# Gautham-JS/ROS_Stereo_SLAM

Hardware: AMD Instinct MI355X
Metric: stereo frames/sec @1241x376, 4096 kpts (higher is better)
Workload: dtype u8/i32 fixed-point (LK) + f32/f64 (geometry)

## Files before the change

ros_stereo_slam_amd/csrc/anms.hip:

```cpp
#include <cfloat>

#include "svo_internal.h"
#include "wave_ops.hip.h"

namespace {


struct AnmsJob {
    const float2 *xy;
    const float *resp;
    int *order;
    float4 *sorted;
    double *radius, *decision;
    int *out_idx, *d_count;
    const float2 *in_a, *in_b;
    float2 *out_a, *out_b;
    const uint8_t *in_s;
    uint8_t *out_s;
    const int *gate;
};
template <int NJ> struct AnmsBatchN {
    AnmsJob j[NJ];
};
using AnmsBatch = AnmsBatchN<SVO_LK_MAX_JOBS>;

constexpr int KPW_GROUP = 8;
constexpr int KPW_LONE = 2;

template <int KPW> __global__ __launch_bounds__(64) void anms_rank_kernel(AnmsBatchN<KPW == KPW_LONE ? 1 : SVO_LK_MAX_JOBS> batch, int n)
{
    svo_chain_priority();
    const AnmsJob &job = batch.j[blockIdx.y];
    if (job.gate && *job.gate == 0)
        return;
    const float2 *__restrict__ xy = job.xy;
    const float *__restrict__ resp = job.resp;
    int *__restrict__ order = job.order;
    float4 *__restrict__ sorted = job.sorted;
    const int lane = threadIdx.x & 63;
    const int i0 = blockIdx.x * KPW;
    if (i0 >= n)
        return;
    float ri[KPW];
    int cnt[KPW];
#pragma unroll
    for (int q = 0; q < KPW; q++) {
        ri[q] = resp[min(i0 + q, n - 1)];
        cnt[q] = 0;
    }
    const float *__restrict__ rl = resp + lane;
    const int own = (i0 >> 6) << 6;
#pragma unroll 2
    for (int j0 = 0; j0 < own; j0 += 64) {
        const float rj = rl[j0];
#pragma unroll
        for (int q = 0; q < KPW; q++)
            cnt[q] += rj >= ri[q] ? 1 : 0;
    }
    {
        const int j = own + lane;
        if (j < n) {
            const float rj = rl[own];
#pragma unroll
            for (int q = 0; q < KPW; q++)
                cnt[q] += (rj > ri[q] || (rj == ri[q] && j < i0 + q)) ? 1 : 0;
        }
    }
    int j0 = own + 64;
#pragma unroll 2
    for (; j0 + 64 <= n; j0 += 64) {
        const float rj = rl[j0];
#pragma unroll
        for (int q = 0; q < KPW; q++)
            cnt[q] += rj > ri[q] ? 1 : 0;
    }
    if (j0 < n && j0 + lane < n) {
        const float rj = rl[j0];
#pragma unroll
        for (int q = 0; q < KPW; q++)
            cnt[q] += rj > ri[q] ? 1 : 0;
    }
#pragma unroll
    for (int q = 0; q < KPW; q++) {
        const int rank = svo::wave_sum_dpp(cnt[q]);
        if (lane == 0 && i0 + q < n) {
            order[rank] = i0 + q;
            const float2 p = xy[i0 + q];
            sorted[rank] = make_float4(p.x, p.y, ri[q], 0.f);
        }
    }
}

template <int KPW> __global__ __launch_bounds__(64) void anms_radius_kernel(AnmsBatchN<KPW == KPW_LONE ? 1 : SVO_LK_MAX_JOBS> batch, int n)
{
    svo_chain_priority();
    if (batch.j[blockIdx.y].gate && *batch.j[blockIdx.y].gate == 0)
        return;
    const float4 *__restrict__ sorted = batch.j[blockIdx.y].sorted;
    double *__restrict__ radius_sq = batch.j[blockIdx.y].radius;
    const int lane = threadIdx.x & 63;
    const int s0 = blockIdx.x * KPW;
    if (s0 >= n)
        return;
    float mx[KPW], my[KPW], thr[KPW];
    double best[KPW];
    unsigned active = 0;
#pragma unroll
    for (int q = 0; q < KPW; q++) {
        const float4 me = sorted[min(s0 + q, n - 1)];
        mx[q] = me.x;
        my[q] = me.y;
        thr[q] = me.z * 1.11f;
        best[q] = DBL_MAX;
        if (s0 + q < n && s0 + q > 0)
            active |= 1u << q;
    }
    for (int j0 = 0; j0 < s0 + KPW - 1 && active; j0 += 64) {
        const int j = j0 + lane;
        const float4 o = sorted[min(j, n - 1)];
#pragma unroll
        for (int q = 0; q < KPW; q++) {
            if (!((active >> q) & 1u))
                continue;
            bool dom = false;
            if (j < s0 + q) {
                dom = o.z > thr[q];
                if (dom) {
                    const float dx = mx[q] - o.x, dy = my[q] - o.y;
                    const double d = (double)dx * dx + (double)dy * dy;
                    best[q] = d < best[q] ? d : best[q];
                }
            }
            if (!__any(dom) || j0 + 64 >= s0 + q)
                active &= ~(1u << q);
        }
    }
#pragma unroll
    for (int q = 0; q < KPW; q++) {
        double b = best[q];
#pragma unroll
        for (int off = 32; off >= 1; off >>= 1) {
            const double o = __shfl_xor(b, off);
            b = o < b ? o : b;
        }
        if (lane == 0 && s0 + q < n)
            radius_sq[s0 + q] = b;
    }
}

template <int KPW> __global__ __launch_bounds__(64) void anms_decide_kernel(AnmsBatchN<KPW == KPW_LONE ? 1 : SVO_LK_MAX_JOBS> batch, int n, int keep)
{
    svo_chain_priority();
    if (batch.j[blockIdx.y].gate && *batch.j[blockIdx.y].gate == 0)
        return;
    const double *__restrict__ radius_sq = batch.j[blockIdx.y].radius;
    double *__restrict__ decision = batch.j[blockIdx.y].decision;
    const int lane = threadIdx.x & 63;
    const int s0 = blockIdx.x * KPW;
    if (s0 >= n)
        return;
    double ri[KPW];
    int gt[KPW], ge[KPW];
#pragma unroll
    for (int q = 0; q < KPW; q++) {
        ri[q] = radius_sq[min(s0 + q, n - 1)];
        gt[q] = ge[q] = 0;
    }
    const double *__restrict__ rl = radius_sq + lane;
    int j0 = 0;
#pragma unroll 2
    for (; j0 + 64 <= n; j0 += 64) {
        const double rj = rl[j0];
#pragma unroll
        for (int q = 0; q < KPW; q++) {
            gt[q] += rj > ri[q] ? 1 : 0;
            ge[q] += rj >= ri[q] ? 1 : 0;
        }
    }
    if (j0 + lane < n) {
        const double rj = rl[j0];
#pragma unroll
        for (int q = 0; q < KPW; q++) {
            gt[q] += rj > ri[q] ? 1 : 0;
            ge[q] += rj >= ri[q] ? 1 : 0;
        }
    }
#pragma unroll
    for (int q = 0; q < KPW; q++) {
        const int g = svo::wave_sum_dpp(gt[q]), e = svo::wave_sum_dpp(ge[q]);
        if (lane == 0 && s0 + q < n && g <= keep && keep < e)
            *decision = ri[q];
    }
}

constexpr int GATHER_T = 256;
template <int NJ> __global__ __launch_bounds__(GATHER_T) void anms_gather_kernel(AnmsBatchN<NJ> batch, int n)
{
    svo_chain_priority();
    const AnmsJob &job = batch.j[blockIdx.x];
    if (job.gate && *job.gate == 0)
        return;
    const double *__restrict__ radius_sq = job.radius;
    const double decision = *job.decision;
    const int *__restrict__ order = job.order;
    int *__restrict__ out_idx = job.out_idx;
    int *__restrict__ d_count = job.d_count;
    __shared__ int s_wave[GATHER_T / 64];
    const int t = threadIdx.x, lane = t & 63, wave = t >> 6;
    const int per = (n + GATHER_T - 1) / GATHER_T;
    const int b = t * per, e = min(b + per, n);
    int cnt = 0;
    for (int i = b; i < e; i++)
        cnt += radius_sq[i] >= decision ? 1 : 0;
    int incl = cnt;
#pragma unroll
    for (int off = 1; off < 64; off <<= 1) {
        const int o = __shfl_up(incl, off, 64);
        incl += lane >= off ? o : 0;
    }
    if (lane == 63)
        s_wave[wave] = incl;
    __syncthreads();
    int pos = incl - cnt, total = 0;
#pragma unroll
    for (int w2 = 0; w2 < GATHER_T / 64; w2++) {
        const int wt = s_wave[w2];
        pos += w2 < wave ? wt : 0;
        total += wt;
    }
    if (t == 0)
        *d_count = total;
    for (int i = b; i < e; i++)
        if (radius_sq[i] >= decision) {
            const int j = order[i];
            out_idx[pos] = j;
            if (job.out_a) {
                job.out_a[pos] = job.in_a[j];
                job.out_b[pos] = job.in_b[j];
                job.out_s[pos] = job.in_s[j];
            }
            pos++;
        }
}

template <int NJ> __global__ __launch_bounds__(64) void anms_payload_kernel(AnmsBatchN<NJ> batch, int n)
{
    const AnmsJob &job = batch.j[blockIdx.y];
    if (job.gate && *job.gate == 0)
        return;
    const int i = blockIdx.x * 64 + threadIdx.x;
    if (i == 0)
        *job.d_count = n;
    if (i >= n)
        return;
    const int j = job.order[i];
    job.out_idx[i] = j;
    if (!job.out_a)
        return;
    job.out_a[i] = job.in_a[j];
    job.out_b[i] = job.in_b[j];
    if (job.out_s)
        job.out_s[i] = job.in_s[j];
}

}

int svo_launch_anms_batch(svo_ctx *ctx, int k, const float *const *xy, const float *const *resp, int n, int keep,
                          int *const *out_idx, int *const *d_count, const svo_anms_gather *gather, const int *const *gates)
{
    if (n <= 0 || k <= 0)
        return SVO_OK;
    if (k > SVO_LK_MAX_JOBS) {
        svo_set_error("anms: at most %d jobs per launch", SVO_LK_MAX_JOBS);
        return SVO_ERR_ARG;
    }
    ScopedKernelTime tm(ctx, SVO_K_ANMS);
    int rc;
    const size_t na = ((size_t)n + 63) / 64 * 64;
    if ((rc = ctx->w_a.ensure(na * 4 * k)) || (rc = ctx->w_b.ensure((na * 8 + 64) * k)) ||
        (rc = ctx->w_d.ensure(na * 16 * k)))
        return rc;
    AnmsBatch batch;
    for (int a = 0; a < SVO_LK_MAX_JOBS; a++) {
        const int q = a < k ? a : 0;
        AnmsJob &j = batch.j[a];
        j.xy = reinterpret_cast<const float2 *>(xy[q]);
        j.resp = resp[q];
        j.order = ctx->w_a.as<int>() + na * q;
        j.radius = reinterpret_cast<double *>(ctx->w_b.as<uint8_t>() + (na * 8 + 64) * q);
        j.decision = j.radius + na;
        j.sorted = ctx->w_d.as<float4>() + na * q;
        j.out_idx = out_idx[q];
        j.d_count = d_count[q];
        j.in_a = gather ? reinterpret_cast<const float2 *>(gather[q].in_a) : nullptr;
        j.in_b = gather ? reinterpret_cast<const float2 *>(gather[q].in_b) : nullptr;
        j.out_a = gather ? reinterpret_cast<float2 *>(gather[q].out_a) : nullptr;
        j.out_b = gather ? reinterpret_cast<float2 *>(gather[q].out_b) : nullptr;
        j.in_s = gather ? gather[q].in_s : nullptr;
        j.out_s = gather ? gather[q].out_s : nullptr;
        j.gate = gates ? gates[q] : nullptr;
    }
    const bool lone = k == 1;
    const int kpw = lone ? KPW_LONE : KPW_GROUP;
    const dim3 wgrid((n + kpw - 1) / kpw, k), block(64);
    AnmsBatchN<1> one;
    one.j[0] = batch.j[0];
    if (lone)
        hipLaunchKernelGGL(anms_rank_kernel<KPW_LONE>, wgrid, block, 0, ctx->stream, one, n);
    else
        hipLaunchKernelGGL(anms_rank_kernel<KPW_GROUP>, wgrid, block, 0, ctx->stream, batch, n);
    if (n <= keep) {
        if (lone)
            hipLaunchKernelGGL(anms_payload_kernel<1>, dim3((n + 63) / 64, k), dim3(64), 0, ctx->stream, one, n);
        else
            hipLaunchKernelGGL(anms_payload_kernel<SVO_LK_MAX_JOBS>, dim3((n + 63) / 64, k), dim3(64), 0, ctx->stream, batch, n);
        SVO_HIP(hipGetLastError());
        return SVO_OK;
    }
    if (lone) {
        hipLaunchKernelGGL(anms_radius_kernel<KPW_LONE>, wgrid, block, 0, ctx->stream, one, n);
        hipLaunchKernelGGL(anms_decide_kernel<KPW_LONE>, wgrid, block, 0, ctx->stream, one, n, keep);
        hipLaunchKernelGGL(anms_gather_kernel<1>, dim3(k), dim3(GATHER_T), 0, ctx->stream, one, n);
    } else {
        hipLaunchKernelGGL(anms_radius_kernel<KPW_GROUP>, wgrid, block, 0, ctx->stream, batch, n);
        hipLaunchKernelGGL(anms_decide_kernel<KPW_GROUP>, wgrid, block, 0, ctx->stream, batch, n, keep);
        hipLaunchKernelGGL(anms_gather_kernel<SVO_LK_MAX_JOBS>, dim3(k), dim3(GATHER_T), 0, ctx->stream, batch, n);
    }
    SVO_HIP(hipGetLastError());
    return SVO_OK;
}

int svo_launch_anms(svo_ctx *ctx, const float *xy, const float *resp, int n, int keep, int *out_idx, int *d_count)
{
    return svo_launch_anms_batch(ctx, 1, &xy, &resp, n, keep, &out_idx, &d_count);
}

extern "C" int svo_anms(svo_ctx *ctx, const float *xy, const float *response, int n, int num_to_keep, int *out_idx,
                        int *count, int mem)
{
    SVO_CHECK_ARG(ctx && n >= 0 && num_to_keep >= 0);
    SVO_CHECK_ARG(mem == SVO_MEM_HOST || mem == SVO_MEM_DEVICE);
    if (n == 0) {
        if (count && mem == SVO_MEM_HOST)
            *count = 0;
        else if (count)
            SVO_HIP(hipMemsetAsync(count, 0, sizeof(int), ctx->stream));
        return SVO_OK;
    }
    SVO_CHECK_ARG(xy && response && out_idx && count);
    if (mem == SVO_MEM_DEVICE)
        return svo_launch_anms(ctx, xy, response, n, num_to_keep, out_idx, count);
    int rc;
    if ((rc = ctx->s_a.ensure((size_t)n * 8)) || (rc = ctx->s_b.ensure((size_t)n * 4)) ||
        (rc = ctx->s_c.ensure((size_t)n * 4 + 64)))
        return rc;
    SVO_HIP(hipMemcpyAsync(ctx->s_a.p, xy, (size_t)n * 8, hipMemcpyHostToDevice, ctx->stream));
    SVO_HIP(hipMemcpyAsync(ctx->s_b.p, response, (size_t)n * 4, hipMemcpyHostToDevice, ctx->stream));
    int *didx = ctx->s_c.as<int>(), *dcnt = didx + n;
    rc = svo_launch_anms(ctx, ctx->s_a.as<float>(), ctx->s_b.as<float>(), n, num_to_keep, didx, dcnt);
    if (rc)
        return rc;
    SVO_HIP(hipMemcpyAsync(ctx->pinned, dcnt, 4, hipMemcpyDeviceToHost, ctx->stream));
    SVO_HIP(hipStreamSynchronize(ctx->stream));
    const int k = *reinterpret_cast<int *>(ctx->pinned);
    SVO_HIP(hipMemcpyAsync(out_idx, didx, (size_t)k * 4, hipMemcpyDeviceToHost, ctx->stream));
    SVO_HIP(hipStreamSynchronize(ctx->stream));
    *count = k;
    return SVO_OK;
}
```

ros_stereo_slam_amd/csrc/context.hip:

```cpp
#include <cstdarg>

#include <cstdlib>
#include <chrono>
#include <cstdlib>
#include <thread>

#include "svo_internal.h"

static thread_local char g_err[512] = "";

void svo_set_error(const char *fmt, ...)
{
    va_list ap;
    va_start(ap, fmt);
    vsnprintf(g_err, sizeof(g_err), fmt, ap);
    va_end(ap);
}

int DevBuf::ensure(size_t bytes)
{
    if (bytes <= cap)
        return SVO_OK;
    if (p)
        (void)hipFree(p);
    p = nullptr;
    cap = 0;
    size_t want = bytes < 4096 ? 4096 : bytes + bytes / 4;
    hipError_t e = hipMalloc(&p, want);
    if (e != hipSuccess) {
        svo_set_error("hipMalloc(%zu) -> %s", want, hipGetErrorString(e));
        return SVO_ERR_HIP;
    }
    cap = want;
    return SVO_OK;
}

void DevBuf::release()
{
    if (p)
        (void)hipFree(p);
    p = nullptr;
    cap = 0;
}

ScopedKernelTime::ScopedKernelTime(svo_ctx *c, int kid) : ctx(c), id(kid)
{
    if (!ctx->timing)
        return;
    KernelTimer &t = ctx->timers[id];
    if (!t.pool.empty()) {
        a = t.pool.back().first;
        b = t.pool.back().second;
        t.pool.pop_back();
    } else {
        if (hipEventCreate(&a) != hipSuccess || hipEventCreate(&b) != hipSuccess) {
            a = b = nullptr;
            return;
        }
    }
    (void)hipEventRecord(a, ctx->stream);
}

ScopedKernelTime::~ScopedKernelTime()
{
    if (!a)
        return;
    (void)hipEventRecord(b, ctx->stream);
    ctx->timers[id].pending.emplace_back(a, b);
}

int svo_resolve_timers(svo_ctx *ctx)
{
    for (int k = 0; k < SVO_K_COUNT; k++) {
        KernelTimer &t = ctx->timers[k];
        for (auto &pr : t.pending) {
            float ms = 0.f;
            if (hipEventSynchronize(pr.second) == hipSuccess &&
                hipEventElapsedTime(&ms, pr.first, pr.second) == hipSuccess) {
                t.total_ms += ms;
                t.launches++;
            }
            t.pool.push_back(pr);
        }
        t.pending.clear();
    }
    return SVO_OK;
}

int svo_wait(svo_ctx *ctx) { return svo_wait_stream(ctx, ctx->stream); }

int svo_wait_stream(svo_ctx *ctx, hipStream_t stream)
{
    static const long spin_us = [] {
        const char *e = getenv("SVO_WAIT_SPIN_US");
        return e ? atol(e) : 300L;
    }();
    SVO_HIP(hipEventRecord(ctx->wait_ev, stream));
    const auto t0 = std::chrono::steady_clock::now();
    for (unsigned n = 0;; n++) {
        hipError_t e = hipEventQuery(ctx->wait_ev);
        if (e == hipSuccess)
            return SVO_OK;
        if (e != hipErrorNotReady) {
            svo_set_error("hipEventQuery -> %s", hipGetErrorString(e));
            return SVO_ERR_HIP;
        }
        if ((n & 15) != 15)
            continue;
        const long us = (long)std::chrono::duration_cast<std::chrono::microseconds>(std::chrono::steady_clock::now() - t0).count();
        if (us < spin_us)
            continue;
        if (us < spin_us + 2000)
            std::this_thread::yield();
        else
            std::this_thread::sleep_for(std::chrono::microseconds(50));
    }
}

extern "C" {

int svo_version(void) { return SVO_VERSION; }
const char *svo_last_error(void) { return g_err; }

int svo_ctx_create(int device, svo_ctx **out)
{
    SVO_CHECK_ARG(out != nullptr);
    *out = nullptr;
    int count = 0;
    hipError_t e = hipGetDeviceCount(&count);
    if (e != hipSuccess || count <= 0) {
        svo_set_error("no HIP device available (%s); libsvo_hip has no CPU fallback",
                      e == hipSuccess ? "device count 0" : hipGetErrorString(e));
        return SVO_ERR_NO_DEVICE;
    }
    SVO_CHECK_ARG(device >= 0 && device < count);
    SVO_HIP(hipSetDevice(device));
    hipDeviceProp_t prop;
    SVO_HIP(hipGetDeviceProperties(&prop, device));
    if (strncmp(prop.gcnArchName, "gfx950", 6) != 0) {
        svo_set_error("device %d is %s; this library carries gfx950 code objects only", device,
                      prop.gcnArchName);
        return SVO_ERR_NO_DEVICE;
    }
    svo_ctx *ctx = new svo_ctx();
    ctx->device = device;
    if (const char *pr = getenv("SVO_CTX_PRIORITY_EXPERIMENT"); pr && atoi(pr)) {
        int lo = 0, hi = 0;
        (void)hipDeviceGetStreamPriorityRange(&lo, &hi);
        e = hipStreamCreateWithPriority(&ctx->stream, hipStreamNonBlocking, atoi(pr) > 0 ? hi : lo);
    } else
        e = hipStreamCreateWithFlags(&ctx->stream, hipStreamNonBlocking);
    if (e != hipSuccess) {
        delete ctx;
        svo_set_error("hipStreamCreate -> %s", hipGetErrorString(e));
        return SVO_ERR_HIP;
    }
    ctx->pinned_bytes = 1 << 16;
    e = hipHostMalloc(&ctx->pinned, ctx->pinned_bytes, hipHostMallocDefault);
    if (e != hipSuccess) {
        (void)hipStreamDestroy(ctx->stream);
        delete ctx;
        svo_set_error("hipHostMalloc -> %s", hipGetErrorString(e));
        return SVO_ERR_HIP;
    }
    if (hipMalloc(reinterpret_cast<void **>(&ctx->d_tickets), SVO_N_TICKETS * sizeof(unsigned)) != hipSuccess ||
        hipMemset(ctx->d_tickets, 0, SVO_N_TICKETS * sizeof(unsigned)) != hipSuccess) {
        (void)hipHostFree(ctx->pinned);
        (void)hipStreamDestroy(ctx->stream);
        delete ctx;
        svo_set_error("hipMalloc(tickets) failed");
        return SVO_ERR_HIP;
    }
    e = hipEventCreateWithFlags(&ctx->wait_ev, hipEventDisableTiming);
    if (e != hipSuccess) {
        (void)hipHostFree(ctx->pinned);
        (void)hipStreamDestroy(ctx->stream);
        delete ctx;
        svo_set_error("hipEventCreate -> %s", hipGetErrorString(e));
        return SVO_ERR_HIP;
    }
    *out = ctx;
    return SVO_OK;
}

int svo_ctx_destroy(svo_ctx *ctx)
{
    if (!ctx)
        return SVO_OK;
    (void)hipSetDevice(ctx->device);
    (void)hipStreamSynchronize(ctx->stream);
    svo_resolve_timers(ctx);
    for (int k = 0; k < SVO_K_COUNT; k++)
        for (auto &pr : ctx->timers[k].pool) {
            (void)hipEventDestroy(pr.first);
            (void)hipEventDestroy(pr.second);
        }
    if (ctx->orb_cache)
        svo_orb_destroy(ctx->orb_cache);
    ctx->orb_cache = nullptr;
    if (ctx->orb_cv_cache)
        svo_orb_cv_destroy(ctx->orb_cv_cache);
    ctx->orb_cv_cache = nullptr;
    DevBuf *bufs[] = {&ctx->s_img, &ctx->s_a, &ctx->s_b, &ctx->s_c, &ctx->s_d, &ctx->s_e,
                      &ctx->s_f,   &ctx->s_g, &ctx->w_a, &ctx->w_b, &ctx->w_c, &ctx->w_d,
                      &ctx->w_e,   &ctx->orb_out, &ctx->orb_cv_out, &ctx->orb_cv_img, &ctx->orb_cv_ptrs,
                      &ctx->sgbm_cost, &ctx->sgbm_misc, &ctx->sgbm_rp, &ctx->sor_grid, &ctx->icp_work, &ctx->ess,
                      &ctx->feat_img, &ctx->feat_sum, &ctx->sift_pyr, &ctx->sift_work, &ctx->sift_out,
                      &ctx->brief_work, &ctx->brief_pat, &ctx->surf_planes, &ctx->surf_work,
                      &ctx->wls_work, &ctx->wls_maps, &ctx->wls_lut, &ctx->fast_work,
                      &ctx->voxel_work, &ctx->voxel_stage, &ctx->rect_stage};
    for (DevBuf *b : bufs)
        b->release();
    ctx->up_ring.release();
    for (int k = 0; k < 3; k++) {
        if (ctx->up_ev[k])
            (void)hipEventDestroy(ctx->up_ev[k]);
        if (ctx->use_ev[k])
            (void)hipEventDestroy(ctx->use_ev[k]);
    }
    if (ctx->up_stream)
        (void)hipStreamDestroy(ctx->up_stream);
    if (ctx->d_tickets)
        (void)hipFree(ctx->d_tickets);
    if (ctx->pinned)
        (void)hipHostFree(ctx->pinned);
    if (ctx->wait_ev)
        (void)hipEventDestroy(ctx->wait_ev);
    (void)hipStreamDestroy(ctx->stream);
    delete ctx;
    return SVO_OK;
}

int svo_ctx_sync(svo_ctx *ctx)
{
    SVO_CHECK_ARG(ctx != nullptr);
    SVO_HIP(hipStreamSynchronize(ctx->stream));
    return SVO_OK;
}

void *svo_ctx_stream(svo_ctx *ctx) { return ctx ? (void *)ctx->stream : nullptr; }

int svo_ctx_enable_kernel_timing(svo_ctx *ctx, int enable)
{
    SVO_CHECK_ARG(ctx != nullptr);
    ctx->timing = enable != 0;
    return SVO_OK;
}

int svo_ctx_kernel_time(svo_ctx *ctx, int kernel_id, double *total_ms, int *launches)
{
    SVO_CHECK_ARG(ctx != nullptr && kernel_id >= 0 && kernel_id < SVO_K_COUNT);
    SVO_HIP(hipStreamSynchronize(ctx->stream));
    svo_resolve_timers(ctx);
    if (total_ms)
        *total_ms = ctx->timers[kernel_id].total_ms;
    if (launches)
        *launches = ctx->timers[kernel_id].launches;
    return SVO_OK;
}

int svo_ctx_reset_kernel_time(svo_ctx *ctx)
{
    SVO_CHECK_ARG(ctx != nullptr);
    SVO_HIP(hipStreamSynchronize(ctx->stream));
    svo_resolve_timers(ctx);
    for (int k = 0; k < SVO_K_COUNT; k++) {
        ctx->timers[k].total_ms = 0;
        ctx->timers[k].launches = 0;
    }
    return SVO_OK;
}

}
```

ros_stereo_slam_amd/csrc/svo_internal.h:

```cpp
#pragma once

#include <hip/hip_runtime.h>

#include <cstdint>
#include <cstdio>
#include <cstring>
#include <string>
#include <vector>

#include "../../include/svo.h"
#include "../../include/svo_math.h"

#define SVO_MAX_LEVELS 4
#define SVO_LK_WIN 21
#define SVO_PYR_PAD 32
#define SVO_LK_MAX_JOBS 16

#define SVO_N_TICKETS 64
static_assert(32 + 2 * SVO_LK_MAX_JOBS <= SVO_N_TICKETS, "svo_ctx::d_tickets: lk_expand_kernel's slots end past the allocation");

void svo_set_error(const char *fmt, ...);

__device__ __forceinline__ void svo_chain_priority() { __builtin_amdgcn_s_setprio(3); }

__host__ __device__ __forceinline__ int svo_bgr2gray(int b, int g, int r) { return (1868 * b + 9617 * g + 4899 * r + 8192) >> 14; }

#define SVO_HIP(call)                                                                         \
    do {                                                                                      \
        hipError_t e_ = (call);                                                               \
        if (e_ != hipSuccess) {                                                               \
            svo_set_error("%s:%d %s -> %s", __FILE__, __LINE__, #call, hipGetErrorString(e_)); \
            return SVO_ERR_HIP;                                                               \
        }                                                                                     \
    } while (0)

#define SVO_CHECK_ARG(cond)                                                  \
    do {                                                                     \
        if (!(cond)) {                                                       \
            svo_set_error("%s:%d bad argument: %s", __FILE__, __LINE__, #cond); \
            return SVO_ERR_ARG;                                              \
        }                                                                    \
    } while (0)

struct PyrDev {
    const uint8_t *lvl[SVO_MAX_LEVELS];
    int pitch[SVO_MAX_LEVELS];
    int w[SVO_MAX_LEVELS];
    int h[SVO_MAX_LEVELS];
    int levels;
    int c;
};

struct Mat34 {
    double m[12];
};

#define SVO_PYR_HEADER 256
enum { SVO_PYR_MONO = 0, SVO_PYR_COLOUR_SEEN = 1, SVO_PYR_STORED = 2, SVO_PYR_COLOUR_VALID = 3 };
__host__ __device__ __forceinline__ int *svo_pyr_words(const uint8_t *padded)
{
    return reinterpret_cast<int *>(const_cast<uint8_t *>(padded) - SVO_PYR_HEADER);
}
__host__ __device__ __forceinline__ int svo_grey_pitch(int w) { return (w + 2 * SVO_PYR_PAD + 15) & ~15; }
__host__ __device__ __forceinline__ int svo_grey_dpitch(int w) { return ((w + 2 * 32 ) * 4 + 15) & ~15; }
__device__ __forceinline__ const uint8_t *svo_pyr_pixel0(const uint8_t *lvl0, int pitch, int c, int w, int gdelta0, int x, int y,
                                                         int *step)
{
    *step = c >= 3 ? 1 : 0;
    if (c == 3) {
        const int *words = svo_pyr_words(lvl0 - (ptrdiff_t)SVO_PYR_PAD * pitch - SVO_PYR_PAD * c);
        if (words[SVO_PYR_STORED] == 1) {
            *step = 0;
            return lvl0 + gdelta0 + (ptrdiff_t)y * svo_grey_pitch(w) + x;
        }
    }
    return lvl0 + (size_t)y * pitch + x * c;
}

struct svo_pyramid {
    int w, h, c, levels;
    uint8_t *base;
    size_t off[SVO_MAX_LEVELS];
    uint8_t *origin(int l) const
    {
        return base + off[l] + (size_t)SVO_PYR_PAD * dev.pitch[l] + (size_t)SVO_PYR_PAD * c;
    }
    size_t bytes;
    PyrDev dev;
    int *dbase = nullptr;
    size_t doff[SVO_MAX_LEVELS] = {0, 0, 0, 0};
    int dpitch[SVO_MAX_LEVELS] = {0, 0, 0, 0};
    size_t goff[SVO_MAX_LEVELS] = {0, 0, 0, 0}, gdoff[SVO_MAX_LEVELS] = {0, 0, 0, 0};
    int gdelta[SVO_MAX_LEVELS] = {0, 0, 0, 0};
    bool want_deriv = true, has_deriv = false;
};
#define SVO_DERIV_PAD 32
int svo_build_derivatives(svo_ctx *ctx, int k, svo_pyramid *const *pyrs);
int svo_expand_grey_storage(svo_ctx *ctx, const svo_pyramid *pyr, bool deriv);
int svo_pyramid_create_ex(svo_ctx *ctx, int width, int height, int channels, int levels, bool want_deriv,
                          svo_pyramid **out);

struct DevBuf {
    void *p = nullptr;
    size_t cap = 0;
    int ensure(size_t bytes);
    void release();
    template <class T> T *as() { return reinterpret_cast<T *>(p); }
};

struct KernelTimer {
    std::vector<std::pair<hipEvent_t, hipEvent_t>> pending;
    std::vector<std::pair<hipEvent_t, hipEvent_t>> pool;
    double total_ms = 0;
    int launches = 0;
};

struct svo_ctx {
    int device = 0;
    hipStream_t stream = nullptr;
    bool timing = false;
    KernelTimer timers[SVO_K_COUNT];
    DevBuf s_img, s_a, s_b, s_c, s_d, s_e, s_f, s_g;
    DevBuf w_a, w_b, w_c, w_d, w_e;
    unsigned *d_tickets = nullptr;
    void *pinned = nullptr;
    size_t pinned_bytes = 0;
    hipEvent_t wait_ev = nullptr;
    struct svo_orb *orb_cache = nullptr;
    int orb_key[5] = {0, 0, 0, 0, 0};
    DevBuf orb_out;
    std::vector<unsigned char> orb_host;
    struct svo_orb_cv *orb_cv_cache = nullptr;
    int orb_cv_key[8] = {0, 0, 0, 0, 0, 0, 0, 0};
    int8_t orb_pattern[1024];
    int has_pattern = 0;
    DevBuf orb_cv_out, orb_cv_img, orb_cv_ptrs;
    hipStream_t up_stream = nullptr;
    DevBuf up_ring;
    hipEvent_t up_ev[3] = {nullptr, nullptr, nullptr}, use_ev[3] = {nullptr, nullptr, nullptr};
    DevBuf sgbm_cost, sgbm_misc, sgbm_rp;
    DevBuf sor_grid;
    DevBuf icp_work;
    DevBuf ess;
    DevBuf feat_img, feat_sum;
    DevBuf sift_pyr, sift_work, sift_out;
    DevBuf brief_work, brief_pat;
    int8_t brief_pattern[3][2048];
    int brief_has_pattern[3] = {0, 0, 0};
    int brief_pat_live[3] = {0, 0, 0};
    DevBuf surf_planes, surf_work;
    DevBuf wls_work, wls_maps, wls_lut;
    std::vector<float> wls_lut_host;
    double wls_lut_sigma = 0;
    int wls_lut_c = 0;
    DevBuf fast_work;
    DevBuf voxel_work, voxel_stage;
    DevBuf rect_stage;
    std::vector<unsigned char> ba_win_host;
};

int svo_wait(svo_ctx *ctx);
int svo_wait_stream(svo_ctx *ctx, hipStream_t stream);

struct ScopedKernelTime {
    svo_ctx *ctx;
    int id;
    hipEvent_t a = nullptr, b = nullptr;
    ScopedKernelTime(svo_ctx *c, int kid);
    ~ScopedKernelTime();
};
int svo_resolve_timers(svo_ctx *ctx);

enum { SVO_HALT_NONE = 0, SVO_HALT_RETRY = 1 ,
       SVO_HALT_FEW_REF = 2  };
struct VoOut {
    double R[9], t[3];
    int inliers, tracked, keyframe, pad;
};
struct VoChain {
    int run;
    int kf;
    int nref;
    int frame;
    int halt_code;
    int kf_n;
    int refine_due;
    int pad;
    double R[9], t[3];
    int kf_min, retry_below;
    float *ref2d, *ref3d;
    VoOut *out;
};

int svo_build_pyramid_from_device(svo_ctx *ctx, svo_pyramid *pyr, const uint8_t *d_image);
int svo_build_pyramids_from_device(svo_ctx *ctx, int k, svo_pyramid *const *pyrs, const uint8_t *const *d_images,
                                   const int *const *gates = nullptr);
struct LkJob {
    PyrDev prev, next;
    const int *dprev;
    const float *prev_pts;
    int n_cap;
    const int *d_n;
    float *next_pts;
    uint8_t *status;
    float *err, *min_eig;
    const int *gate = nullptr;
};
template <int NJ> struct LkBatchN {
    LkJob j[NJ];
};
using LkBatch = LkBatchN<SVO_LK_MAX_JOBS>;
int svo_launch_lk_batch(svo_ctx *ctx, int n_jobs, const LkJob *jobs, const svo_pyramid *geom);
int svo_launch_lk(svo_ctx *ctx, svo_pyramid *prev, const svo_pyramid *next, const float *prev_pts,
                  int n, float *next_pts, uint8_t *status, float *err, float *min_eig,
                  const int *d_n = nullptr);
int svo_launch_grid(svo_ctx *ctx, int rows, int cols, int step, float *out_xy, int cap);

struct svo_compact_job {
    const uint8_t *mask;
    int cap;
    const int *d_n;
    const float *in[3];
    float *out[3];
    int stride[3];
    int *d_count;
    const int *gate = nullptr;
    const int *alt_sel = nullptr;
    const uint8_t *alt_mask = nullptr;
    const float *alt_in[3] = {nullptr, nullptr, nullptr};
    const int *alt_d_n = nullptr;
};
struct svo_fransac_job {
    const float *p1, *p2;
    int cap;
    const int *d_n;
    double threshold, confidence;
    int max_iters;
    uint64_t seed;
    uint8_t *mask;
    double *d_F;
    int *d_count, *d_iters;
    const svo_compact_job *then_compact = nullptr;
    const int *gate = nullptr;
    int gate_stride = 0;
    bool cv_small = true;
};
int svo_launch_fransac_batch(svo_ctx *ctx, int n_jobs, const svo_fransac_job *jobs);
int svo_launch_fransac(svo_ctx *ctx, const float *p1, const float *p2, int cap, const int *d_n,
                       double threshold, double confidence, int max_iters, uint64_t seed, uint8_t *mask,
                       double *d_F, int *d_count, int *d_iters, const svo_compact_job *then_compact = nullptr,
                       bool cv_small = true);
int svo_fransac_ex(svo_ctx *ctx, const float *p1, const float *p2, int n, double threshold, double confidence, int max_iters,
                   uint64_t seed, uint8_t *mask, double *F9, int *inlier_count, int *iters_run, int mem, bool cv_small);
int svo_launch_triangulate(svo_ctx *ctx, const double *P1, const double *P2, const float *x1, const float *x2,
                           int cap, const int *d_n, float *out_xyz, float *out_h, const double *Rt,
                           float *out_world);
struct svo_tri_job {
    const float *x1, *x2;
    int cap;
    const int *d_n;
    float *out_xyz, *out_h;
    const double *Rt;
    float *out_world;
    int *h_count;
    VoChain *chain = nullptr;
    float *out_x1 = nullptr;
    const svo_pyramid *color_src = nullptr;
    float *color_out = nullptr;
};
int svo_launch_triangulate_batch(svo_ctx *ctx, const double *P1, const double *P2, int k, const svo_tri_job *jobs);
int svo_launch_keyframe_place(svo_ctx *ctx, VoChain *chain, const float *x1, const float *xyz, int cap, const int *d_n,
                              float *out_x1, float *out_cam, float *out_world, const svo_pyramid *color_src, float *color_out,
                              int what);
int svo_launch_transform(svo_ctx *ctx, const double *Rt, const float *in, int cap, const int *d_n, float *out);
int svo_launch_colors(svo_ctx *ctx, const svo_pyramid *pyr, const float *xy, int cap, const int *d_n, float *out);
int svo_launch_compact_batch(svo_ctx *ctx, int n_jobs, const svo_compact_job *jobs);
int svo_launch_compact(svo_ctx *ctx, const uint8_t *mask, int cap, const int *d_n, const float *in_a, int stride_a,
                       float *out_a, const float *in_b, int stride_b, float *out_b, const float *in_c, int stride_c,
                       float *out_c, int *d_count);
struct svo_orb;
int svo_orb_create(svo_ctx *ctx, int w, int h, int c, int n_features, int fast_t, svo_orb **out);
int svo_orb_destroy(svo_orb *o);
int svo_orb_launch(svo_orb *o, const uint8_t *d_image, float *d_xy, int *d_oct, float *d_resp, float *d_dir,
                   uint32_t *d_desc, int *d_n);
struct svo_orb_cv;
int svo_orb_cv_create(svo_ctx *ctx, int w, int h, int c, int n_features, int fast_t, int n_levels, float scale_factor, int batch,
                      const int8_t *pattern, svo_orb_cv **out);
int svo_orb_cv_destroy(svo_orb_cv *o);
int svo_orb_cv_set_pattern(svo_orb_cv *o, const int8_t *pattern);
int svo_orb_cv_batch(const svo_orb_cv *o);
int svo_orb_cv_launch(svo_orb_cv *o, const uint8_t *const *d_images, int n_images, int cap_out, float *d_xy, int *d_oct,
                      float *d_resp, float *d_dir, uint32_t *d_desc, int *d_n, hipStream_t st);
void svo_orb_default_pattern(int8_t *pat);
int svo_launch_sor(svo_ctx *ctx, const float *xyz, const float *color, int cap, int mean_k, double stddev_mul,
                   float z_limit, float *xyz_out, float *color_out, int *d_count, float *d_mean_dist, int *d_pass);
int svo_launch_sor_large(svo_ctx *ctx, const float *xyz, const float *color, int cap, int mean_k, double stddev_mul,
                         float z_limit, float *xyz_out, float *color_out, int *d_count, float *d_mean_dist, int *d_pass);
struct svo_pnp_job {
    const float *obj, *img;
    int cap;
    const int *d_n;
    double K4[4];
    int iterations;
    double reproj_err, confidence;
    uint64_t seed;
    int refine_iters;
    int *inliers;
    uint8_t *mask;
    void *d_result;
    VoChain *chain = nullptr;
    const int *cnt_trk;
};
int svo_launch_pnp_ransac_batch(svo_ctx *ctx, int n_jobs, const svo_pnp_job *jobs, bool split);
int svo_launch_pnp_refine(svo_ctx *ctx, int n_jobs, const svo_pnp_job *jobs, bool keyframes);
int svo_launch_pnp_ransac_batch(svo_ctx *ctx, int n_jobs, const svo_pnp_job *jobs);
int svo_launch_pnp_ransac(svo_ctx *ctx, const float *obj, const float *img, int cap, const int *d_n,
                          const double *K4h, int iterations, double reproj_err, double confidence, uint64_t seed,
                          int refine_iters, int *inliers, uint8_t *mask, void *d_result);
int svo_launch_solve_pnp(svo_ctx *ctx, const float *obj, const float *img, int cap, const int *d_n, const double *K4h,
                         int refine_iters, int *inliers, void *d_result);
struct svo_anms_gather {
    const float *in_a, *in_b;
    float *out_a, *out_b;
    const uint8_t *in_s;
    uint8_t *out_s;
};
int svo_launch_anms_batch(svo_ctx *ctx, int k, const float *const *xy, const float *const *resp, int n, int keep,
                          int *const *out_idx, int *const *d_count, const svo_anms_gather *gather = nullptr,
                          const int *const *gates = nullptr);
int svo_launch_anms(svo_ctx *ctx, const float *xy, const float *resp, int n, int keep, int *out_idx, int *d_count);

const char *svo_png_info(const uint8_t *data, size_t n, int *w, int *h, int *c);
const char *svo_png_decode(const uint8_t *data, size_t n, int channels, uint8_t *out, size_t cap, int *w, int *h);

struct svo_voc;
constexpr int SVO_LC_MAX_CAND = 64;
struct svo_lc_bow_record {
    int ready;
    int nq;
    int n_cand, n_feat;
    double last_sum;
    int cand_id[SVO_LC_MAX_CAND];
    double cand_sum[SVO_LC_MAX_CAND];
};
int svo_voc_launch_transform(svo_voc *v, hipStream_t st, const uint32_t *d_desc, int cap, const int *d_n, int levelsup,
                             int *d_word, double *d_weight, int *d_node, int n_frames = 1);
int svo_bow_launch_vector(hipStream_t st, const int *d_word, const double *d_weight, const int *d_node, int cap, const int *d_n,
                          int *row_w, double *row_v, int *row_n, int *row_node, int n_frames = 1);
int svo_bow_launch_query(hipStream_t st, const int *qw, const double *qv, const int *d_nq, int nf, const int *head,
                         const int *next, const double *db_v, int stride, int n_entries, double *plane, int pitch, double *sums,
                         int dislocal, int k_want, int entry_id, const int *d_nfeat, svo_lc_bow_record *rec, int n_frames, unsigned *mask);
inline int svo_bow_mask_words(int nf) { return ((nf + 127) / 128) * 4; }
int svo_bow_launch_link(hipStream_t st, const int *row_w, const int *row_n, int nf, int slot0, int *head, int *next, int n_frames = 1);
struct SvoDiBatch {
    int old_entry[SVO_LK_MAX_JOBS], cur_entry[SVO_LK_MAX_JOBS], na[SVO_LK_MAX_JOBS];
};
int svo_bow_launch_di_nearest_batch(hipStream_t st, const SvoDiBatch &b, int n_checks, int na_max, const uint32_t *db_desc,
                                    const int *db_node, const int *db_n, int nf, uint8_t *out, size_t out_stride);
int svo_bow_launch_di_nearest(hipStream_t st, const uint32_t *A, const int *node_a, int na, const uint32_t *B, const int *node_b,
                              const int *d_nb, int *best_j, int *d1, int *d2);
int svo_voc_words_internal(const svo_voc *v);
int svo_voc_device_internal(const svo_voc *v);
int svo_voc_levels_internal(const svo_voc *v);
```

Before: 14000.

## Accelerate ANMS radius search with a spatial hash grid and ring-bounded lookups

The rank kernel now writes each keypoint's sorted rank once per lane and, when suppression is needed, scatters keypoints into a 32px spatial hash grid of capped cells. The radius kernel scans only the first stripes of stronger points linearly, then looks up nearby grid cells ring by ring and stops once the best distance is under the ring bound, instead of scanning all stronger points. The decide kernel clears the grid counters for the next call. This adds atomics, an overflow flag that falls back to the linear scan, and a persistent grid buffer per job.

```diff
diff --git a/ros_stereo_slam_amd/csrc/anms.hip b/ros_stereo_slam_amd/csrc/anms.hip
--- a/ros_stereo_slam_amd/csrc/anms.hip
+++ b/ros_stereo_slam_amd/csrc/anms.hip
@@ -1,5 +1,6 @@
 #include <cfloat>
 
+#include "anms_grid_plan.hip.h"
 #include "svo_internal.h"
 #include "wave_ops.hip.h"
 
@@ -18,6 +19,7 @@
     const uint8_t *in_s;
     uint8_t *out_s;
     const int *gate;
+    int *grid;
 };
 template <int NJ> struct AnmsBatchN {
     AnmsJob j[NJ];
@@ -27,7 +29,8 @@
 constexpr int KPW_GROUP = 8;
 constexpr int KPW_LONE = 2;
 
-template <int KPW> __global__ __launch_bounds__(64) void anms_rank_kernel(AnmsBatchN<KPW == KPW_LONE ? 1 : SVO_LK_MAX_JOBS> batch, int n)
+template <int KPW> __global__ __launch_bounds__(64) void anms_rank_kernel(AnmsBatchN<KPW == KPW_LONE ? 1 : SVO_LK_MAX_JOBS> batch, int n,
+                                                                          int fill)
 {
     svo_chain_priority();
     const AnmsJob &job = batch.j[blockIdx.y];
@@ -80,42 +83,41 @@
         for (int q = 0; q < KPW; q++)
             cnt[q] += rj > ri[q] ? 1 : 0;
     }
-#pragma unroll
-    for (int q = 0; q < KPW; q++) {
-        const int rank = svo::wave_sum_dpp(cnt[q]);
-        if (lane == 0 && i0 + q < n) {
-            order[rank] = i0 + q;
-            const float2 p = xy[i0 + q];
-            sorted[rank] = make_float4(p.x, p.y, ri[q], 0.f);
-        }
-    }
-}
-
-template <int KPW> __global__ __launch_bounds__(64) void anms_radius_kernel(AnmsBatchN<KPW == KPW_LONE ? 1 : SVO_LK_MAX_JOBS> batch, int n)
-{
-    svo_chain_priority();
-    if (batch.j[blockIdx.y].gate && *batch.j[blockIdx.y].gate == 0)
-        return;
-    const float4 *__restrict__ sorted = batch.j[blockIdx.y].sorted;
-    double *__restrict__ radius_sq = batch.j[blockIdx.y].radius;
-    const int lane = threadIdx.x & 63;
-    const int s0 = blockIdx.x * KPW;
-    if (s0 >= n)
-        return;
-    float mx[KPW], my[KPW], thr[KPW];
-    double best[KPW];
-    unsigned active = 0;
-#pragma unroll
-    for (int q = 0; q < KPW; q++) {
-        const float4 me = sorted[min(s0 + q, n - 1)];
-        mx[q] = me.x;
-        my[q] = me.y;
-        thr[q] = me.z * 1.11f;
-        best[q] = DBL_MAX;
-        if (s0 + q < n && s0 + q > 0)
-            active |= 1u << q;
-    }
-    for (int j0 = 0; j0 < s0 + KPW - 1 && active; j0 += 64) {
+    int rank = 0;
+#pragma unroll
+    for (int q = 0; q < KPW; q++) {
+        const int r = svo::wave_sum_dpp(cnt[q]);
+        rank = lane == q ? r : rank;
+    }
+    if (lane >= KPW || i0 + lane >= n)
+        return;
+    const int i = i0 + lane;
+    order[rank] = i;
+    const float2 p = xy[i];
+    const float r = resp[i];
+    sorted[rank] = make_float4(p.x, p.y, r, 0.f);
+    if (!fill)
+        return;
+    namespace ag = anms_grid;
+    int *__restrict__ grid = job.grid;
+    int cx, cy;
+    const bool okx = ag::cell_of(p.x, &cx), oky = ag::cell_of(p.y, &cy);
+    int pos = ag::CAP;
+    const int e = ag::entry_of(cx, cy);
+    if (okx && oky)
+        pos = atomicAdd(grid + e, 1);
+    if (pos < ag::CAP)
+        reinterpret_cast<float4 *>(grid + ag::SLOTS_AT)[e * ag::CAP + pos] = make_float4(p.x, p.y, r, __int_as_float(rank));
+    else
+        grid[ag::FLAG_AT] = 1;
+}
+
+template <int KPW>
+__device__ __forceinline__ void anms_scan_stripes(const float4 *__restrict__ sorted, int n, int s0, int lane, int j_begin, int j_end,
+                                                  const float (&mx)[KPW], const float (&my)[KPW], const float (&thr)[KPW],
+                                                  double (&best)[KPW], unsigned &active)
+{
+    for (int j0 = j_begin; j0 < j_end && active; j0 += 64) {
         const int j = j0 + lane;
         const float4 o = sorted[min(j, n - 1)];
 #pragma unroll
@@ -135,6 +137,105 @@
                 active &= ~(1u << q);
         }
     }
+}
+
+template <int KPW> __global__ __launch_bounds__(64) void anms_radius_kernel(AnmsBatchN<KPW == KPW_LONE ? 1 : SVO_LK_MAX_JOBS> batch, int n)
+{
+    namespace ag = anms_grid;
+    constexpr int G = 64 / KPW;
+    static_assert(G >= 8 && G <= ag::CAP && (G & (G - 1)) == 0, "lane sub of a group preloads the counter of ring 1's cell sub");
+    svo_chain_priority();
+    if (batch.j[blockIdx.y].gate && *batch.j[blockIdx.y].gate == 0)
+        return;
+    const float4 *__restrict__ sorted = batch.j[blockIdx.y].sorted;
+    double *__restrict__ radius_sq = batch.j[blockIdx.y].radius;
+    const int *__restrict__ grid = batch.j[blockIdx.y].grid;
+    const int lane = threadIdx.x & 63;
+    const int s0 = blockIdx.x * KPW;
+    if (s0 >= n)
+        return;
+    float mx[KPW], my[KPW], thr[KPW];
+    double best[KPW];
+    unsigned active = 0;
+#pragma unroll
+    for (int q = 0; q < KPW; q++) {
+        const float4 me = sorted[min(s0 + q, n - 1)];
+        mx[q] = me.x;
+        my[q] = me.y;
+        thr[q] = me.z * 1.11f;
+        best[q] = DBL_MAX;
+        if (s0 + q < n && s0 + q > 0)
+            active |= 1u << q;
+    }
+    const int j_end = s0 + KPW - 1;
+    anms_scan_stripes<KPW>(sorted, n, s0, lane, 0, min(j_end, ag::STRIPES * 64), mx, my, thr, best, active);
+    if (active && grid[ag::FLAG_AT] == 0) {
+        const float4 *__restrict__ slots = reinterpret_cast<const float4 *>(grid + ag::SLOTS_AT);
+        const int g = lane / G, sub = lane % G;
+        float gx = 0.f, gy = 0.f, gthr = 0.f;
+#pragma unroll
+        for (int q = 0; q < KPW; q++)
+            if (g == q)
+                gx = mx[q], gy = my[q], gthr = thr[q];
+        const int gs = s0 + g;
+        bool live = (active >> g) & 1u;
+        int cx, cy;
+        ag::cell_of(gx, &cx);
+        ag::cell_of(gy, &cy);
+        double gb = DBL_MAX;
+        auto visit = [&](int e, int c) {
+            for (int s = sub; s < c; s += G) {
+                const float4 o = slots[e * ag::CAP + s];
+                if (o.z > gthr && __float_as_int(o.w) < gs) {
+                    const float dx = gx - o.x, dy = gy - o.y;
+                    const double d = (double)dx * dx + (double)dy * dy;
+                    gb = d < gb ? d : gb;
+                }
+            }
+        };
+        const int e0 = ag::entry_of(cx, cy);
+        int c0 = 0, c1 = 0, e1 = 0;
+        if (live) {
+            c0 = min(grid[e0], ag::CAP);
+            if (sub < 8) {
+                int dx, dy;
+                ag::ring_cell(1, sub, &dx, &dy);
+                e1 = ag::entry_of(cx + dx, cy + dy);
+                c1 = min(grid[e1], ag::CAP);
+            }
+        }
+        visit(e0, c0);
+#pragma unroll
+        for (int t = 0; t < 8; t++)
+            visit(__shfl(e1, g * G + t), __shfl(c1, g * G + t));
+        for (int r = 1;; r++) {
+            double m = gb;
+#pragma unroll
+            for (int off = G / 2; off >= 1; off >>= 1) {
+                const double o = __shfl_xor(m, off);
+                m = o < m ? o : m;
+            }
+            live = live && !(m <= ag::ring_bound(r));
+            if (r == ag::RINGS || !__any(live))
+                break;
+            const int nc = ag::ring_cells(r + 1);
+            for (int t = 0; t < nc; t++) {
+                int dx, dy;
+                ag::ring_cell(r + 1, t, &dx, &dy);
+                const int e = ag::entry_of(cx + dx, cy + dy);
+                visit(e, live ? min(grid[e], ag::CAP) : 0);
+            }
+        }
+        const unsigned long long lv = __ballot(live);
+#pragma unroll
+        for (int q = 0; q < KPW; q++) {
+            if (g == q)
+                best[q] = gb < best[q] ? gb : best[q];
+            if (!((lv >> (q * G)) & 1ull))
+                active &= ~(1u << q);
+        }
+    }
+    anms_scan_stripes<KPW>(sorted, n, s0, lane, ag::STRIPES * 64, j_end, mx, my, thr, best, active);
 #pragma unroll
     for (int q = 0; q < KPW; q++) {
         double b = best[q];
@@ -156,6 +257,8 @@
     const double *__restrict__ radius_sq = batch.j[blockIdx.y].radius;
     double *__restrict__ decision = batch.j[blockIdx.y].decision;
     const int lane = threadIdx.x & 63;
+    for (int c = blockIdx.x * 64 + lane; c <= anms_grid::CELLS; c += gridDim.x * 64)
+        batch.j[blockIdx.y].grid[c] = 0;
     const int s0 = blockIdx.x * KPW;
     if (s0 >= n)
         return;
@@ -280,6 +383,15 @@
     if ((rc = ctx->w_a.ensure(na * 4 * k)) || (rc = ctx->w_b.ensure((na * 8 + 64) * k)) ||
         (rc = ctx->w_d.ensure(na * 16 * k)))
         return rc;
+    if (n > keep && ctx->anms_cells_jobs < k) {
+        ctx->anms_cells_jobs = 0;
+        if ((rc = ctx->anms_cells.ensure(anms_grid::JOB_BYTES * k)))
+            return rc;
+        for (int a = 0; a < k; a++)
+            SVO_HIP(hipMemsetAsync(ctx->anms_cells.as<uint8_t>() + anms_grid::JOB_BYTES * a, 0, anms_grid::SLOTS_AT * sizeof(int),
+                                   ctx->stream));
+        ctx->anms_cells_jobs = k;
+    }
     AnmsBatch batch;
     for (int a = 0; a < SVO_LK_MAX_JOBS; a++) {
         const int q = a < k ? a : 0;
@@ -299,6 +411,7 @@
         j.in_s = gather ? gather[q].in_s : nullptr;
         j.out_s = gather ? gather[q].out_s : nullptr;
         j.gate = gates ? gates[q] : nullptr;
+        j.grid = n > keep ? reinterpret_cast<int *>(ctx->anms_cells.as<uint8_t>() + anms_grid::JOB_BYTES * q) : nullptr;
     }
     const bool lone = k == 1;
     const int kpw = lone ? KPW_LONE : KPW_GROUP;
@@ -306,9 +419,9 @@
     AnmsBatchN<1> one;
     one.j[0] = batch.j[0];
     if (lone)
-        hipLaunchKernelGGL(anms_rank_kernel<KPW_LONE>, wgrid, block, 0, ctx->stream, one, n);
+        hipLaunchKernelGGL(anms_rank_kernel<KPW_LONE>, wgrid, block, 0, ctx->stream, one, n, n > keep ? 1 : 0);
     else
-        hipLaunchKernelGGL(anms_rank_kernel<KPW_GROUP>, wgrid, block, 0, ctx->stream, batch, n);
+        hipLaunchKernelGGL(anms_rank_kernel<KPW_GROUP>, wgrid, block, 0, ctx->stream, batch, n, n > keep ? 1 : 0);
     if (n <= keep) {
         if (lone)
             hipLaunchKernelGGL(anms_payload_kernel<1>, dim3((n + 63) / 64, k), dim3(64), 0, ctx->stream, one, n);
diff --git a/ros_stereo_slam_amd/csrc/anms_grid_plan.hip.h b/ros_stereo_slam_amd/csrc/anms_grid_plan.hip.h
--- /dev/null
+++ b/ros_stereo_slam_amd/csrc/anms_grid_plan.hip.h
@@ -0,0 +1,62 @@
+#pragma once
+
+#include <cstddef>
+#include <cstdint>
+
+#ifdef __HIPCC__
+#define ANMS_GRID_HD __host__ __device__
+#else
+#define ANMS_GRID_HD
+#endif
+
+namespace anms_grid {
+
+constexpr int S = 32;
+constexpr int HX_BITS = 6, HY_BITS = 4;
+constexpr int HX = 1 << HX_BITS, HY = 1 << HY_BITS;
+constexpr int CELLS = HX * HY;
+constexpr int CAP = 32;
+constexpr int RINGS = 3;
+constexpr int STRIPES = 2;
+constexpr float COORD_MAX = 1048576.f;
+
+constexpr int FLAG_AT = CELLS;
+constexpr int SLOTS_AT = CELLS + 64;
+constexpr size_t JOB_INTS = (size_t)SLOTS_AT + (size_t)CELLS * CAP * 4;
+constexpr size_t JOB_BYTES = JOB_INTS * 4;
+static_assert(SLOTS_AT % 4 == 0 && JOB_BYTES % 16 == 0, "the slots are read as float4");
+
+ANMS_GRID_HD inline bool cell_of(float v, int *c)
+{
+    if (!(v >= -COORD_MAX && v <= COORD_MAX)) {
+        *c = 0;
+        return false;
+    }
+    int i = (int)(v * (1.0f / S));
+    if ((float)(i * S) > v)
+        i--;
+    *c = i;
+    return true;
+}
+
+ANMS_GRID_HD inline int entry_of(int cx, int cy) { return (cx & (HX - 1)) | ((cy & (HY - 1)) << HX_BITS); }
+
+ANMS_GRID_HD inline double ring_bound(int r) { return (double)(r * S) * (double)(r * S); }
+
+ANMS_GRID_HD inline int ring_cells(int r) { return r == 0 ? 1 : 8 * r; }
+ANMS_GRID_HD inline void ring_cell(int r, int t, int *dx, int *dy)
+{
+    if (r == 0) {
+        *dx = *dy = 0;
+        return;
+    }
+    const int side = 2 * r, e = t / side, o = t - e * side;
+    switch (e) {
+    case 0: *dx = -r + o, *dy = -r; break;
+    case 1: *dx = r, *dy = -r + o; break;
+    case 2: *dx = r - o, *dy = r; break;
+    default: *dx = -r, *dy = r - o; break;
+    }
+}
+
+}
diff --git a/ros_stereo_slam_amd/csrc/context.hip b/ros_stereo_slam_amd/csrc/context.hip
--- a/ros_stereo_slam_amd/csrc/context.hip
+++ b/ros_stereo_slam_amd/csrc/context.hip
@@ -208,7 +208,7 @@
                       &ctx->feat_img, &ctx->feat_sum, &ctx->sift_pyr, &ctx->sift_work, &ctx->sift_out,
                       &ctx->brief_work, &ctx->brief_pat, &ctx->surf_planes, &ctx->surf_work,
                       &ctx->wls_work, &ctx->wls_maps, &ctx->wls_lut, &ctx->fast_work,
-                      &ctx->voxel_work, &ctx->voxel_stage, &ctx->rect_stage};
+                      &ctx->voxel_work, &ctx->voxel_stage, &ctx->rect_stage, &ctx->anms_cells};
     for (DevBuf *b : bufs)
         b->release();
     ctx->up_ring.release();
diff --git a/ros_stereo_slam_amd/csrc/svo_internal.h b/ros_stereo_slam_amd/csrc/svo_internal.h
--- a/ros_stereo_slam_amd/csrc/svo_internal.h
+++ b/ros_stereo_slam_amd/csrc/svo_internal.h
@@ -156,6 +156,8 @@
     DevBuf fast_work;
     DevBuf voxel_work, voxel_stage;
     DevBuf rect_stage;
+    DevBuf anms_cells;
+    int anms_cells_jobs = 0;
     std::vector<unsigned char> ba_win_host;
 };
 
```

Measured after the change: 14040 (median of 6 runs). No clear change (+0.3%).
